# microsoft/protnote

Hardware: AMD Instinct MI355X
Metric: protein-label pairs/sec (fwd+bwd) (higher is better)
Workload: dtype f32

## Files before the change

### include/protnote_hip.h

```cpp
#ifndef PROTNOTE_HIP_H
#define PROTNOTE_HIP_H

#include <stddef.h>
#include <stdint.h>

#ifdef __cplusplus
extern "C" {
#endif

#define PN_MAX_BLOCKS 16
#define PN_MAX_LAYERS 8
#define PN_LABEL_F32 0
#define PN_LABEL_I64 1
#define PN_LABEL_U8 2

const char* pn_last_error(void);
int pn_version(void);
const char* pn_build_hash(void);

typedef struct pn_bn {
  const float* weight;
  const float* bias;
  float* running_mean;
  float* running_var;
// ... 214 lines not shown

int pn_set_mlp_materialize(int on);

typedef int (*pn_sync_hook)(long n_doubles, void* user);
int pn_set_sync_bn(pn_sync_hook hook, void* user, double* stage, long stage_doubles, int world);
int pn_get_math_mode(void);

int pn_set_backward_math(int mode);
int pn_get_backward_math(void);

int pn_set_forward_math(int mode);
int pn_get_forward_math(void);
int pn_set_fwd_staged(int on);
int pn_set_bf16_mfma16(int on);
int pn_set_bwd_deep(int mask);

int pn_set_f32_dma(int on);
int pn_set_b3_dma(int on);

int pn_set_encoder_f64(int on);

int pn_set_conv1_gather(int on);

int pn_dropout_mask(unsigned seed, int stream, float p, long rows, int cols, float* out, void* stream_);

int pn_prof_begin(void);
int pn_prof_end(int max_kinds, int* kinds, long* counts, double* total_ms, double* total_flops);

size_t pn_gemm_nt_stats_ws_bytes(int M, int N);
int pn_gemm_nt(const float* A, long lda, const float* W, long ldw, float* C, long ldc, int M, int N, int K,
// ... 8 lines not shown
```

### protnote_amd/__init__.py

```python
__version__ = "0.1.0"


def free_workspaces():
    from . import _lib

    _lib._ws_cache.clear()


def set_math_mode(mode) -> None:
    from . import _lib

    _lib.set_math_mode(mode)


def get_math_mode() -> str:
    from . import _lib

    return _lib.get_math_mode()


def set_backward_math(mode) -> None:
    from . import _lib

    _lib.set_backward_math(mode)
# ... 5 lines not shown
    return _lib.get_backward_math()


def set_forward_math(mode) -> None:
    from . import _lib

    _lib.set_forward_math(mode)


def get_forward_math() -> str:
    from . import _lib

    return _lib.get_forward_math()


_PROTNOTE_ALIASES = {
    "protnote": "protnote_amd",
    "protnote.models": "protnote_amd.models",
    "protnote.models.ProtNote": "protnote_amd.models.ProtNote",
    "protnote.models.protein_encoders": "protnote_amd.models.protein_encoders",
    "protnote.models.ProtNoteTrainer": "protnote_amd.models.ProtNoteTrainer",
    "protnote.utils": "protnote_amd.utils",
    "protnote.utils.losses": "protnote_amd.utils.losses",
    "protnote.utils.models": "protnote_amd.utils.models",
    "protnote.utils.configs": "protnote_amd.utils.configs",
    "protnote.utils.proteinfer": "protnote_amd.utils.proteinfer",
    "protnote.utils.evaluation": "protnote_amd.utils.evaluation",
    "protnote.data": "protnote_amd.data",
    "protnote.data.collators": "protnote_amd.data.collators",
    "protnote.data.samplers": "protnote_amd.data.samplers",
# ... 22 lines not shown
```

### protnote_amd/_lib.py

```python
import ctypes as C
import os

import torch

_HERE = os.path.dirname(os.path.abspath(__file__))
LIB_PATH = os.path.join(_HERE, "libprotnote_hip.so")

PN_MAX_BLOCKS = 16
PN_MAX_LAYERS = 8
PN_ADAM_WS_BYTES = 32768
fp = C.POINTER(C.c_float)


class pn_bn(C.Structure):
    _fields_ = [("weight", C.c_void_p), ("bias", C.c_void_p), ("running_mean", C.c_void_p),
                ("running_var", C.c_void_p)]


class pn_res_block(C.Structure):
    _fields_ = [("bn1", pn_bn), ("conv_a_w", C.c_void_p), ("conv_a_b", C.c_void_p), ("bn2", pn_bn),
                ("conv_b_w", C.c_void_p), ("conv_b_b", C.c_void_p)]


class pn_encoder(C.Structure):
# ... 142 lines not shown
                                        C.c_void_p, C.c_int, C.c_void_p, C.c_void_p, C.c_void_p]),
    "pn_binned_auprc": (C.c_int, [C.c_void_p, C.c_void_p, C.c_int, C.c_int, C.c_void_p, C.c_void_p, C.c_int,
                                  C.c_void_p]),
    "pn_dropout_mask": (C.c_int, [C.c_uint, C.c_int, C.c_float, C.c_long, C.c_int, C.c_void_p, C.c_void_p]),
    "pn_set_math_mode": (C.c_int, [C.c_int]),
    "pn_set_mlp_materialize": (C.c_int, [C.c_int]),
    "pn_set_sync_bn": (C.c_int, [C.c_void_p, C.c_void_p, C.c_void_p, C.c_long, C.c_int]),
    "pn_get_math_mode": (C.c_int, []),
    "pn_set_backward_math": (C.c_int, [C.c_int]),
    "pn_get_backward_math": (C.c_int, []),
    "pn_set_forward_math": (C.c_int, [C.c_int]),
    "pn_get_forward_math": (C.c_int, []),
    "pn_set_fwd_staged": (C.c_int, [C.c_int]),
    "pn_set_bf16_mfma16": (C.c_int, [C.c_int]),
    "pn_set_bwd_deep": (C.c_int, [C.c_int]),
    "pn_set_f32_dma": (C.c_int, [C.c_int]),
    "pn_set_encoder_f64": (C.c_int, [C.c_int]),
    "pn_set_conv1_gather": (C.c_int, [C.c_int]),
    "pn_set_b3_dma": (C.c_int, [C.c_int]),
    "pn_prof_begin": (C.c_int, []),
    "pn_prof_end": (C.c_int, [C.c_int, C.POINTER(C.c_int), C.POINTER(C.c_long), C.POINTER(C.c_double),
                              C.POINTER(C.c_double)]),
    "pn_gemm_nt": (C.c_int, [C.c_void_p, C.c_long, C.c_void_p, C.c_long, C.c_void_p, C.c_long, C.c_int, C.c_int,
                             C.c_int, C.c_void_p, C.c_void_p, C.c_void_p, C.c_void_p, C.c_void_p, C.c_int,
                             C.c_void_p, C.c_size_t, C.c_void_p]),
    "pn_gemm_nt_stats_ws_bytes": (C.c_size_t, [C.c_int, C.c_int]),
    "pn_loss_ws_bytes": (C.c_size_t, [C.c_int, C.c_int]),
}


# ... 58 lines not shown


def get_math_mode() -> str:
    return "bf16x3" if lib().pn_get_math_mode() == 1 else "f32"


def math_field(mode=None) -> int:
    if mode is None:
        return 1 + int(lib().pn_get_math_mode())
    key = str(mode).lower()
    if key not in _MATH_MODES:
        raise ValueError(f"math mode must be 'f32' or 'bf16x3', got {mode!r}")
    return 1 + _MATH_MODES[key]


_BWD_MODES = {"same": 0, "0": 0, "bf16": 1, "1": 1}


def set_backward_math(mode) -> None:
    key = str(mode).lower()
    if key not in _BWD_MODES:
        raise ValueError(f"backward math must be 'same' or 'bf16', got {mode!r}")
    check(lib().pn_set_backward_math(_BWD_MODES[key]))


def get_backward_math() -> str:
    return "bf16" if lib().pn_get_backward_math() == 1 else "same"


def backward_math_field(mode=None) -> int:
# ... 89 lines not shown
```

### protnote_amd/csrc/abi_heads_train.hpp

```cpp
struct MlpSave {
  float* Y[PN_MAX_LAYERS];
  float* H[PN_MAX_LAYERS];
  float *s[PN_MAX_LAYERS], *t[PN_MAX_LAYERS], *mean[PN_MAX_LAYERS], *invstd[PN_MAX_LAYERS];
};

static bool mlp_save_carve(const pn_mlp* m, int rows, Bump& bp, MlpSave& s) {
  for (int l = 0; l + 1 < m->nlayers; ++l) {
    const int h = m->dims[l + 1];
    s.Y[l] = bp.take<float>((size_t)rows * h);
    s.H[l] = m->dropout_p > 0.f ? bp.take<float>((size_t)rows * h) : nullptr;
    s.s[l] = bp.take<float>(h);
    s.t[l] = bp.take<float>(h);
    s.mean[l] = bp.take<float>(h);
    s.invstd[l] = bp.take<float>(h);
  }
  return bp.ok;
}

struct MlpTrainWs {
  double *S1, *S2;
  float *cs, *p, *q, *G[2], *WT, *part;
  size_t part_floats;
  ColScr colscr;
  StatScr statscr;
// ... 244 lines not shown
struct PairTrainWs {
  double *sumA, *sqA, *sumB, *sqB, *S1, *S2, *dwacc, *scal, *s12;
  float *cs, *p, *q, *WT, *weff, *dweff, *part, *dA1, *dB1;
  float* m1part;
  int m1_chunks;
  float* dwpart;
  long dwpart_rows;
  size_t part_floats;
  ColScr colscr;
  StatScr statscr;
  uint16_t* wsplit;
  int* tnsync;
  uint16_t* hbf;
};
static const long PAIR_STATS_ROWS = 4096;
static const int SUM_BLOCKS = 1024;

static bool pair_train_ws_carve(const pn_pairhead* hd, int B, int NL, Bump& bp, PairTrainWs& w) {
  const int h = hd->h, d = hd->d;
  w.sumA = bp.take<double>(h);
  w.sqA = bp.take<double>(h);
  w.sumB = bp.take<double>(h);
  w.sqB = bp.take<double>(h);
  w.S1 = bp.take<double>(h);
  w.S2 = bp.take<double>(h);
  w.dwacc = bp.take<double>(h);
  w.scal = bp.take<double>(4 + SUM_BLOCKS);
  w.s12 = bp.take<double>(2 * (size_t)h);
  w.cs = bp.take<float>(h);
  w.p = bp.take<float>(h);
  w.q = bp.take<float>(h);
  const size_t wt = (size_t)h * (h > 2 * d ? h : 2 * d);
  w.WT = bp.take<float>(wt);
  w.weff = hd->fusion == 1 ? bp.take<float>((size_t)h * 2 * d) : nullptr;
  w.dweff = hd->fusion == 1 ? bp.take<float>((size_t)h * 2 * d) : nullptr;
  w.part_floats = (size_t)16 * h * h < TN_PART_FLOATS_MAX ? (size_t)16 * h * h : TN_PART_FLOATS_MAX;
  w.part = bp.take<float>(w.part_floats);
  w.dA1 = bp.take<float>((size_t)B * h);
  w.dB1 = bp.take<float>((size_t)NL * h);
  w.m1_chunks = (NL + 255) / 256;
  if (w.m1_chunks < 1) w.m1_chunks = 1;
  if (w.m1_chunks > 128) w.m1_chunks = 128;
  w.m1part = (B <= 256 && hd->fusion != 2) ? bp.take<float>((size_t)w.m1_chunks * B * h) : nullptr;
  w.dwpart_rows = w.m1part != nullptr ? w.m1_chunks : NL;
  w.dwpart = (hd->nlayers == 1 && hd->fusion != 2) ? bp.take<float>((size_t)w.dwpart_rows * h) : nullptr;
  colscr_carve(bp, (long)B * NL, h, w.colscr);
  statscr_carve(bp, (long)B * NL, PAIR_STATS_ROWS, h, w.statscr);
  w.wsplit = (uint16_t*)bp.take<float>((size_t)h * h);
  w.tnsync = bp.take<int>(TN_SYNC_INTS);
  w.hbf = nullptr;
  if (fwd_bf16_requested(hd) && fwd_staged_shape(h) && hd->nlayers > 1) {
    const long R = (long)B * NL;
    w.hbf = (uint16_t*)bp.take<float>((size_t)(R < FWD_H_ROWS ? R : FWD_H_ROWS) * h / 2);
  }
  return bp.ok;
}

static long pair_chunk_rows(int B, int NL, int label_chunk) {
  long c = label_chunk <= 0 ? 256 : label_chunk;
  if (c > NL) c = NL;
  return c * (long)B;
// ... 197 lines not shown
  if (!pair_train_ws_carve(hd, B, NL, bw, w)) return fail("pairhead bwd: workspace too small");

  if (gr->db_out != nullptr) {
    hipLaunchKernelGGL(k_sum, dim3(SUM_BLOCKS), dim3(256), 0, st, dl_pairs, R, w.scal + 4);
    hipLaunchKernelGGL(k_scalar_final, dim3(1), dim3(256), 0, st, (const double*)(w.scal + 4), SUM_BLOCKS, w.scal);
    hipLaunchKernelGGL(k_d2f, dim3(1), dim3(64), 0, st, (const double*)w.scal, gr->db_out, 1, 1.f);
    HIP_OK(hipGetLastError());
  }

  const float* G = nullptr;
  const long stats_rows = PAIR_STATS_ROWS;
  if (hd->backward_math < 0 || hd->backward_math > 2)
    return fail("pairhead bwd: backward_math %d (0 = library default, 1 = as the forward, 2 = bf16)", hd->backward_math);
  const int bwd_math = hd->backward_math == 0 ? g_bwd_math.load(std::memory_order_relaxed) : hd->backward_math - 1;
  BwdBf16Scope bwd_scope(bwd_math == 1 && hd->dropout_p == 0.f);
  for (int l = n - 1; l >= 1; --l) {
    const bool top = (l == n - 1);
    float* z = sv.zbuf[l] + (size_t)S * h;
    StatsParams sp;
    memset(&sp, 0, sizeof(sp));
    sp.R = R; sp.C = h; sp.rows_per_block = stats_rows; sp.pairB = 1;
    sp.Z = z; sp.ldz = h;
    sp.s = sv.s[l]; sp.t = sv.t[l]; sp.mean = sv.mean[l]; sp.invstd = sv.invstd[l];
    sp.part = w.statscr.part;
    const dim3 sg(nblk(h, 1024), nblk(R, stats_rows));
    if (top) {
      sp.gvec = dl_pairs; sp.w = hd->w_out;
      {
        ProfScope ps(ST_BN_BWD_STATS, (double)R * (4.0 * h + 4.0), st);
        hipLaunchKernelGGL((k_bn_bwd_stats<1, 0>), sg, dim3(256), 0, st, sp);
      }
      PN_OK(reduce_parts<double>(w.statscr.part, sg.y, 3 * h, h, w.S1, w.S2, w.dwacc, w.statscr.red, st));
    } else {
      sp.G = G; sp.ldg = h;
      {
        ProfScope ps(ST_BN_BWD_STATS, (double)R * 8.0 * h, st);
        hipLaunchKernelGGL((k_bn_bwd_stats<0, 0>), sg, dim3(256), 0, st, sp);
      }
      PN_OK(reduce_parts<double>(w.statscr.part, sg.y, 2 * h, h, w.S1, w.S2, nullptr, w.statscr.red, st));
    }
    PN_OK(bwd_finalize(st, (const double*)w.S1,
                       (const double*)w.S2, (const double*)(top ? w.dwacc : nullptr), (double)R, h,
                       hd->bn[l].weight, (const float*)sv.s[l], (const float*)sv.mean[l],
                       (const float*)sv.invstd[l], top ? hd->w_out : (const float*)nullptr, w.cs, w.p, w.q,
                       gr->dgamma[l], gr->dbeta[l], top ? gr->dw_out : (float*)nullptr));
    HIP_OK(hipGetLastError());

    const bool dz_bf16 = tl_bwd_bf16 && (g_bwd_deep & 4) && h % 256 == 0 && h <= 4096 && R % 32 == 0 && R >= 65536 &&
// ... 26 lines not shown
    tp.A = dz; tp.lda = h;
    const DropSpec ds_in = drop_spec(hd->dropout_p, hd->dropout_seed, DROP_STREAM_PAIR + (l - 1));
    tp.drop_seed = ds_in.seed; tp.drop_thresh = ds_in.thresh; tp.drop_scale = ds_in.scale;
    if (gr->dw[l] == nullptr) {
    } else if (l == 1 && hd->fusion != 2) {
      tp.B = sv.Ap; tp.ldb = h; tp.B2 = sv.Bp; tp.ldb2 = h; tp.pairB = B;
      PN_OK((launch_tn<TA_PLAIN, TB_PAIRSUM_RELU>(tp, gr->dw[l], h, w.part, w.part_floats, st)));
    } else {
      tp.B = sv.zbuf[l - 1] + (size_t)S * h; tp.ldb = h; tp.b_s = sv.s[l - 1]; tp.b_t = sv.t[l - 1];
      tp.task_sync = w.tnsync;
      PN_OK((launch_tn<TA_PLAIN, TB_AFFINE_RELU>(tp, gr->dw[l], h, w.part, w.part_floats, st)));
    }

    PN_OK(transpose_into(hd->w[l], h, h, h, w.WT, h, st));
    const long step = top ? S : R;
    for (long r0 = 0; r0 < R; r0 += step) {
      const long rows = (R - r0 < step) ? R - r0 : step;
      GemmParams p = gp_zero();
      p.M = (int)rows; p.N = h; p.Nstore = h; p.Kseg = h;
      p.A = dz + (size_t)r0 * h; p.lda = h;
      p.W = w.WT; p.ldw = h; p.wsplit = w.wsplit;
      p.C = sv.zbuf[l] + (size_t)r0 * h; p.ldc = h;
      PN_OK((launch_gemm<A_PLAIN, E_STORE>(p, 0, st)));
    }
    tl_dz_bf16 = false;
    G = sv.zbuf[l];
    if (hd->dropout_p > 0.f)
      PN_OK(launch_dropout<0>(G, h, sv.zbuf[l], h, R, h, nullptr, nullptr, ds_in, st));
  }

  tl_bwd_bf16 = false;
  const bool prod = hd->fusion == 2;
  float* dQ = nullptr;
  if (!prod) {
    PairRedParams rp;
    memset(&rp, 0, sizeof(rp));
    rp.B = B; rp.NL = NL; rp.C = h; rp.DH = G; rp.ldh = h;
    rp.A = sv.A1; rp.lda = h; rp.Bm = sv.B1; rp.ldb = h;
    rp.s = sv.s[0]; rp.t = sv.t[0];
// ... 157 lines not shown
```

### protnote_amd/csrc/gemm_bf16_m16.hpp

```cpp
#pragma once
#include "bwd_bf16_dz.hpp"

namespace pn {

__device__ __forceinline__ void st16(float* ptr, float a, float b, float c, float d) {
  *reinterpret_cast<float4*>(ptr) = make_float4(a, b, c, d);
}

__device__ __forceinline__ float dpp_quad(float v, bool xor2) {
  const int x = __builtin_bit_cast(int, v);
  return __builtin_bit_cast(float, xor2 ? __builtin_amdgcn_update_dpp(x, x, 0x4E, 0xF, 0xF, false)
                                        : __builtin_amdgcn_update_dpp(x, x, 0xB1, 0xF, 0xF, false));
}
__device__ __forceinline__ void quad_transpose(float (&x)[4], int a) {
  const bool o1 = a & 1, o2 = a & 2;
  float r0 = dpp_quad(o1 ? x[0] : x[1], false), r1 = dpp_quad(o1 ? x[2] : x[3], false);
  if (o1) { x[0] = r0; x[2] = r1; } else { x[1] = r0; x[3] = r1; }
  r0 = dpp_quad(o2 ? x[0] : x[2], true);
  r1 = dpp_quad(o2 ? x[1] : x[3], true);
  if (o2) { x[0] = r0; x[1] = r1; } else { x[2] = r0; x[3] = r1; }
}

template <int EK, int WAVES_M, int WAVES_N, int FM, int FN>
__device__ __forceinline__ void gemm_epilogue_m16(const GemmParams& p, f32x4 (&acc)[FM][FN], int row0, int col0, int tile_n, float* smem) {
  static_assert(EK == E_STORE || EK == E_ROWDOT, "E_STORE_H16 takes the swapped roles");
  static_assert(FN % 4 == 0, "stores transpose four fragments at a time");
  constexpr int NT = WAVES_M * WAVES_N * 64;
  constexpr int BN = WAVES_N * FN * 16;
  const int tid = threadIdx.x;
  const int lane = tid & 63;
  const int wave = tid >> 6;
  const int wm = wave / WAVES_N;
  const int wn = wave % WAVES_N;
  const int rq = lane >> 4;
  const int cl = lane & 15;
  const int qa = lane & 3, qc = cl >> 2;
  const bool want_stats = (EK == E_STORE) && (p.col_part != nullptr);
  const bool store_act = (EK == E_STORE) && (p.e_scale != nullptr);
  float* red = smem;

  if constexpr (EK == E_ROWDOT) {
    float rowacc[FM][4];
#pragma unroll
    for (int i = 0; i < FM; ++i)
#pragma unroll
      for (int e = 0; e < 4; ++e) rowacc[i][e] = 0.f;
#pragma unroll
    for (int j = 0; j < FN; ++j) {
      const int col = col0 + (wn * FN + j) * 16 + cl;
      const float es = p.e_scale[col], et = p.e_shift[col], ew = p.e_w[col];
#pragma unroll
      for (int i = 0; i < FM; ++i)
// ... 7 lines not shown
        float v = rowacc[i][e];
        v += __shfl_xor(v, 1);
        v += __shfl_xor(v, 2);
        v += __shfl_xor(v, 4);
        v += __shfl_xor(v, 8);
        const int row = row0 + (wm * FM + i) * 16 + 4 * rq + e;
        if (cl == 0 && row < p.M) p.rowdot_out[(long)(tile_n * WAVES_N + wn) * p.M + row] = v;
      }
    }
    return;
  } else {
#pragma unroll
    for (int j = 0; j < FN; ++j) {
      const int col = col0 + (wn * FN + j) * 16 + cl;
      float bj = 0.f, es = 1.f, et = 0.f;
      if constexpr (EK == E_STORE) bj = p.bias ? p.bias[col] : 0.f;
      const bool act = store_act;
      if (act) {
        es = p.e_scale[col];
        et = p.e_shift[col];
      }
      float s1 = 0.f, s2 = 0.f;
#pragma unroll
      for (int i = 0; i < FM; ++i) {
#pragma unroll
        for (int e = 0; e < 4; ++e) {
          float v = acc[i][j][e];
          if constexpr (EK == E_STORE) v += bj;
          if (act) v = relu(fmaf(v, es, et));
          acc[i][j][e] = v;
          const int row = row0 + (wm * FM + i) * 16 + 4 * rq + e;
          if (row < p.M) {
            s1 += v;
            s2 += v * v;
          }
        }
      }
      if (want_stats) {
        s1 += __shfl_xor(s1, 16);
        s2 += __shfl_xor(s2, 16);
        s1 += __shfl_xor(s1, 32);
        s2 += __shfl_xor(s2, 32);
        if (rq == 0) {
          red[(wm * 2 + 0) * BN + (wn * FN + j) * 16 + cl] = s1;
          red[(wm * 2 + 1) * BN + (wn * FN + j) * 16 + cl] = s2;
        }
      }
    }
#pragma unroll
    for (int i = 0; i < FM; ++i) {
#pragma unroll
      for (int e = 0; e < 4; ++e) {
// ... 190 lines not shown
```

### protnote_amd/csrc/gemm_engine.hpp

```cpp
#pragma once
#include <hip/hip_runtime.h>
#include <stdint.h>

#include <type_traits>

#ifndef PN_MINW
#define PN_MINW 2
#endif
#ifndef PN_BK
#define PN_BK 32
#endif
#ifndef PN_XCD
#define PN_XCD 1
#endif

namespace pn {

typedef float f32x16 __attribute__((ext_vector_type(16)));

enum { A_PLAIN = 0, A_AFFINE_RELU = 1, A_PAIRSUM_RELU = 2, A_CONV = 3, A_DZ_ELEM = 4, A_DZ_ROWG = 5, A_PAIRPROD = 6 };
enum { E_STORE = 0, E_CONV = 1, E_ROWDOT = 2, E_SCALE_RC = 3, E_PAIRADD = 4, E_STORE_H16 = 5 };

struct GemmParams {
  int M, N;
  int Nstore;
  int nseg, Kseg;
  const float* A;
  long lda;
  const float* a_scale;
  const float* a_shift;
  const float* A2;
  long lda2;
  int pairB;
  const int* lens;
  int L;
  int dil;
// ... 17 lines not shown
  float alpha;
  const float* gvec;
  const float* dz_cs;
  const float* dz_p;
  const float* dz_q;
  const float* padd1;
  long ldp1;
  const float* padd2;
  long ldp2;
  uint32_t drop_seed, drop_thresh;
  float drop_scale;
  uint16_t* wsplit;
  const uint16_t* w_hi;
  const uint16_t* w_lo;
  int xcd_br, xcd_bc;
  const int* run_if;
};

__device__ __forceinline__ float4 ld4(const float* p) { return *reinterpret_cast<const float4*>(p); }
__device__ __forceinline__ float relu(float x) { return fmaxf(x, 0.f); }

__host__ __device__ __forceinline__ uint32_t pn_lowbias32(uint32_t x) {
  x ^= x >> 16;
  x *= 0x7feb352dU;
  x ^= x >> 15;
  x *= 0x846ca68bU;
  x ^= x >> 16;
  return x;
}
__host__ __device__ __forceinline__ uint32_t drop_rowkey(uint32_t seed, uint32_t row) {
// ... 37 lines not shown
  return true;
}

template <int EK, int WAVES_M, int WAVES_N, int WM, int WN>
__device__ __forceinline__ void gemm_epilogue(const GemmParams& p, f32x16 (&acc)[WM][WN], int row0, int col0, int tile_n,
                                              float* smem) {
  constexpr int NT = WAVES_M * WAVES_N * 64;
  constexpr int BN = WAVES_N * WN * 32;
  const int tid = threadIdx.x;
  const int lane = tid & 63;
  const int wave = tid >> 6;
  const int wm = wave / WAVES_N;
  const int wn = wave % WAVES_N;
  const int hl = lane >> 5;
  const int cl = lane & 31;
  const bool want_stats = (EK == E_STORE || EK == E_CONV || EK == E_PAIRADD) && (p.col_part != nullptr);
  float* red = smem;

  unsigned live_mask[WM];
  if constexpr (EK == E_CONV) {
#pragma unroll
    for (int i = 0; i < WM; ++i) {
      live_mask[i] = 0u;
#pragma unroll
      for (int e = 0; e < 16; ++e) {
        const int row = row0 + (wm * WM + i) * 32 + (e & 3) + 8 * (e >> 2) + 4 * hl;
        const int rc = row < p.M ? row : p.M - 1;
        const int b = rc / p.L;
        const bool live = (row < p.M) && (rc - b * p.L) < p.lens[b];
        live_mask[i] |= (live ? 1u : 0u) << e;
      }
    }
  }

#pragma unroll
  for (int j = 0; j < WN; ++j) {
    const int col = col0 + (wn * WN + j) * 32 + cl;
    const bool cok = col < p.N;
    float s1 = 0.f, s2 = 0.f;
    float bj = 0.f, es = 0.f, et = 0.f, ew = 0.f, cs = 0.f;
    if constexpr (EK == E_STORE || EK == E_CONV || EK == E_PAIRADD) {
      bj = (cok && p.bias) ? p.bias[col] : 0.f;
    }
    if constexpr (EK == E_ROWDOT) {
      if (cok) {
        es = p.e_scale[col];
        et = p.e_shift[col];
        ew = p.e_w[col];
      }
    }
    if constexpr (EK == E_STORE_H16) {
      if (cok) {
        es = p.e_scale[col];
        et = p.e_shift[col];
      }
    }
    const bool store_act = (EK == E_STORE) && (p.e_scale != nullptr);
// ... 16 lines not shown
          const int rc = row < p.M ? row : p.M - 1;
          res[e] = has_res ? p.resid[(long)rc * p.ldr + cc] : 0.f;
        }
#pragma unroll
        for (int e = 0; e < 16; ++e) {
          const int row = row0 + (wm * WM + i) * 32 + (e & 3) + 8 * (e >> 2) + 4 * hl;
          const bool live = (live_mask[i] >> e) & 1u;
          float v = acc[i][j][e];
          v = (live && cok) ? (v + bj) + res[e] : 0.f;
          if (row < p.M && col < p.Nstore) p.C[(long)row * p.ldc + col] = v;
          s1 += v;
          s2 += v * v;
        }
      }
    }
    if constexpr (EK != E_CONV) {
#pragma unroll
    for (int i = 0; i < WM; ++i) {
#pragma unroll
      for (int e = 0; e < 16; ++e) {
        const int row = row0 + (wm * WM + i) * 32 + (e & 3) + 8 * (e >> 2) + 4 * hl;
        const bool rok = row < p.M;
        float v = acc[i][j][e];
        if constexpr (EK == E_PAIRADD) {
          if (rok && cok) {
            const int pj = row / p.pairB;
            const int pi = row - pj * p.pairB;
            v += bj + p.padd1[(long)pi * p.ldp1 + col] + p.padd2[(long)pj * p.ldp2 + col];
            p.C[(long)row * p.ldc + col] = v;
            s1 += v;
            s2 += v * v;
// ... 350 lines not shown
```

### protnote_amd/csrc/protnote_hip.hip

```cpp
#include <hip/hip_runtime.h>
#include <stdarg.h>
#include <stdio.h>
#include <stdlib.h>
#include <string.h>

#include "../../include/protnote_hip.h"
#include "common.hpp"
#include "gemm_engine.hpp"
#include "gemm_bf16x3.hpp"
#include "gemm_bf16.hpp"
#include "gemm_dma.hpp"
#include "gemm_conv_dma.hpp"
#include "gemm_conv_f64.hpp"
#include "gemm_tn_fast.hpp"
#include "train_kernels.hpp"
#include "bwd_bf16_dz.hpp"
#include "fwd_bf16_h.hpp"
#include "gemm_bf16_m16.hpp"

using namespace pn;

static thread_local char g_err[512] = "";

static int fail(const char* fmt, ...) {
// ... 233 lines not shown
  *count_dev = nullptr;
  if (!sync_bn_on()) return 0;
  if (2 * n + 2 > g_sync_cap) return fail("sync_bn: %ld statistics exceed the staging buffer (%ld doubles)", 2 * n + 2, g_sync_cap);
  HIP_OK(hipMemcpyAsync(g_sync_stage, a, n * sizeof(double), hipMemcpyDeviceToDevice, st));
  HIP_OK(hipMemcpyAsync(g_sync_stage + n, b, n * sizeof(double), hipMemcpyDeviceToDevice, st));
  hipLaunchKernelGGL(k_set_double, dim3(1), dim3(1), 0, st, g_sync_stage + 2 * n, local_count);
  if (g_sync_hook(2 * n + 1, g_sync_user) != 0) return fail("sync_bn: the all-reduce callback failed");
  HIP_OK(hipMemcpyAsync(a, g_sync_stage, n * sizeof(double), hipMemcpyDeviceToDevice, st));
  HIP_OK(hipMemcpyAsync(b, g_sync_stage + n, n * sizeof(double), hipMemcpyDeviceToDevice, st));
  double* keep = g_sync_stage + g_sync_cap - 1;
  HIP_OK(hipMemcpyAsync(keep, g_sync_stage + 2 * n, sizeof(double), hipMemcpyDeviceToDevice, st));
  *count_dev = keep;
  return 0;
}

template <int AK, int EK, int WAVES_M, int WAVES_N, int WM, int WN, int BK, bool DROP = false>
static int launch_gemm_cfg(const GemmParams& p, hipStream_t st) {
  using Cfg = GemmCfg<WAVES_M, WAVES_N, WM, WN, BK>;
  auto kern = gemm_nt_kernel<AK, EK, WAVES_M, WAVES_N, WM, WN, BK, DROP>;
  static std::atomic<bool> attr_done[64];
  int dev = 0;
  HIP_OK(hipGetDevice(&dev));
  if (dev < 64 && !attr_done[dev]) {
    HIP_OK(hipFuncSetAttribute((const void*)kern, hipFuncAttributeMaxDynamicSharedMemorySize,
                               Cfg::LDS_BYTES));
    attr_done[dev] = true;
  }
  if (p.M <= 0 || p.Nstore <= 0) return 0;
  if (p.Kseg % 4 != 0) return fail("gemm: K segment %d not a multiple of 4", p.Kseg);
  const long tm = (p.M + Cfg::BM - 1) / Cfg::BM;
  const long tn = (p.Nstore + Cfg::BN - 1) / Cfg::BN;
  if (tm * tn > 0x7fffffffL) return fail("gemm: grid too large");
  GemmParams pp = p;
  const int resident = (Cfg::BM * Cfg::BN >= 256 * 256) ? 32 : 64;
  pp.xcd_bc = (PN_XCD && tm >= 16) ? ((tn % 8 == 0) ? 8 : ((tn % 4 == 0) ? 4 : 0)) : 0;
  if (AK == A_PAIRSUM_RELU && resident == 32 && pp.xcd_bc && tm >= 64) pp.xcd_bc = 1;
  pp.xcd_br = pp.xcd_bc ? resident / pp.xcd_bc : 0;
  long grid = tm * tn;
  if (pp.xcd_bc) {
    const long nblk = ((tm + pp.xcd_br - 1) / pp.xcd_br) * (tn / pp.xcd_bc);
    grid = ((nblk + 7) / 8) * 8 * resident;
  }
  if (grid > 0x7fffffffL) return fail("gemm: grid too large");
  {
    ProfScope ps(AK * 10 + EK, 2.0 * (double)p.M * (double)p.N * (double)p.nseg * (double)p.Kseg, st);
    hipLaunchKernelGGL(kern, dim3((unsigned)grid), dim3(Cfg::NT), Cfg::LDS_BYTES, st, pp);
  }
  HIP_OK(hipGetLastError());
  return finish_col_stats(p, tm, st);
}

static std::atomic<int> g_math_mode{0};
extern "C" int pn_set_math_mode(int mode) {
  if (mode != 0 && mode != 1) return fail("pn_set_math_mode: 0 (f32) or 1 (bf16x3)");
  g_math_mode = mode;
  return 0;
}
extern "C" int pn_get_math_mode(void) { return g_math_mode; }
static thread_local int tl_math = -1;
static inline int cur_math() { return tl_math >= 0 ? tl_math : g_math_mode.load(std::memory_order_relaxed); }
// ... 77 lines not shown
  }
  if (p.M <= 0 || p.Nstore <= 0) return 0;
  if (p.Kseg % 4 != 0) return fail("gemm: K segment %d not a multiple of 4", p.Kseg);
  const long tm = (p.M + Cfg::BM - 1) / Cfg::BM;
  const long tn = (p.Nstore + Cfg::BN - 1) / Cfg::BN;
  GemmParams pp = p;
  pp.xcd_bc = (PN_XCD && tm >= 16) ? ((tn % 8 == 0) ? 8 : ((tn % 4 == 0) ? 4 : 0)) : 0;
  if (!GEN && AK == A_PAIRSUM_RELU && pp.xcd_bc && tm >= 64) pp.xcd_bc = 1;
  pp.xcd_br = pp.xcd_bc ? 32 / pp.xcd_bc : 0;
  long grid = tm * tn;
  if (pp.xcd_bc) {
    const long nblk = ((tm + pp.xcd_br - 1) / pp.xcd_br) * (tn / pp.xcd_bc);
    grid = ((nblk + 7) / 8) * 8 * 32;
  }
  if (grid > 0x7fffffffL) return fail("gemm: grid too large");
  if constexpr (BDMA) {
    pp.w_hi = p.wsplit;
    pp.w_lo = p.wsplit + (size_t)p.N * p.Kseg;
    hipLaunchKernelGGL(k_split_planes, dim3(nblk((long)p.N * p.Kseg / 4, 256)), dim3(256), 0, st, p.W, p.ldw, p.N, p.Kseg,
                       p.wsplit, p.wsplit + (size_t)p.N * p.Kseg);
  }
  {
    ProfScope ps((NP == 3 ? 1000 : 1500) + AK * 10 + EK, 2.0 * (double)p.M * (double)p.N * (double)p.nseg * (double)p.Kseg, st);
    hipLaunchKernelGGL(kern, dim3((unsigned)grid), dim3(Cfg::NT), LDS_BYTES, st, pp);
  }
  HIP_OK(hipGetLastError());
  return finish_col_stats(p, tm, st);
}

static std::atomic<int> g_bwd_deep{7};
extern "C" int pn_set_bwd_deep(int mask) {
  g_bwd_deep = mask & 7;
  return 0;
}
static int launch_gemm_bf16_single(const GemmParams& p, hipStream_t st) {
  auto kern = gemm_nt_bf16_kernel<E_STORE>;
  static std::atomic<bool> attr_done[64];
  int dev = 0;
  HIP_OK(hipGetDevice(&dev));
  if (dev < 64 && !attr_done[dev]) {
    HIP_OK(hipFuncSetAttribute((const void*)kern, hipFuncAttributeMaxDynamicSharedMemorySize, NT_BF16_LDS_BYTES));
    attr_done[dev] = true;
  }
  if (p.M <= 0 || p.Nstore <= 0) return 0;
  const long tm = (p.M + 255) / 256, tn = p.N / 256;
  GemmParams pp = p;
  pp.xcd_bc = (PN_XCD && tm >= 16) ? ((tn % 8 == 0) ? 8 : ((tn % 4 == 0) ? 4 : 0)) : 0;
  pp.xcd_br = pp.xcd_bc ? 32 / pp.xcd_bc : 0;
  long grid = tm * tn;
  if (pp.xcd_bc) {
    const long nblk_ = ((tm + pp.xcd_br - 1) / pp.xcd_br) * (tn / pp.xcd_bc);
    grid = ((nblk_ + 7) / 8) * 8 * 32;
  }
  if (grid > 0x7fffffffL) return fail("gemm: grid too large");
  pp.w_hi = p.wsplit;
  pp.w_lo = p.wsplit + (size_t)p.N * p.Kseg;
  hipLaunchKernelGGL(k_split_planes, dim3(nblk((long)p.N * p.Kseg / 4, 256)), dim3(256), 0, st, p.W, p.ldw, p.N, p.Kseg,
                     p.wsplit, p.wsplit + (size_t)p.N * p.Kseg);
  {
    ProfScope ps(1500 + A_PLAIN * 10 + E_STORE, 2.0 * (double)p.M * (double)p.N * (double)p.Kseg, st);
    hipLaunchKernelGGL(kern, dim3((unsigned)grid), dim3(512), NT_BF16_LDS_BYTES, st, pp);
  }
  HIP_OK(hipGetLastError());
  return 0;
}

static std::atomic<int> g_bf16_m16{1};
extern "C" int pn_set_bf16_mfma16(int on) {
  g_bf16_m16 = on ? 1 : 0;
  return 0;
}
template <int EK>
static int bf16dma_kernel(void (**out)(GemmParams)) {
  static std::atomic<bool> attr_done[64];
  int dev = 0;
  HIP_OK(hipGetDevice(&dev));
  if (dev < 64 && !attr_done[dev]) {
    HIP_OK(hipFuncSetAttribute((const void*)gemm_nt_bf16dma_kernel<EK>, hipFuncAttributeMaxDynamicSharedMemorySize, NT_BF16DMA_LDS_BYTES));
    HIP_OK(hipFuncSetAttribute((const void*)gemm_nt_bf16m16_kernel<EK>, hipFuncAttributeMaxDynamicSharedMemorySize, NT_BF16DMA_LDS_BYTES));
    attr_done[dev] = true;
  }
  *out = g_bf16_m16.load() ? gemm_nt_bf16m16_kernel<EK> : gemm_nt_bf16dma_kernel<EK>;
  return 0;
}

static int launch_gemm_bf16dma(const GemmParams& p, hipStream_t st) {
  void (*kern)(GemmParams) = nullptr;
  if (int rc = bf16dma_kernel<E_STORE>(&kern)) return rc;
  if (p.M <= 0 || p.Nstore <= 0) return 0;
  if (p.wsplit == nullptr || p.Kseg % 64 != 0 || p.N % 256 != 0 || p.Nstore != p.N || (long)256 * p.lda * 4 >= (1L << 32) ||
      (long)256 * p.Kseg * 2 >= (1L << 32))
    return fail("gemm (bf16 dz): shape %d x %d x %d not supported", p.M, p.N, p.Kseg);
  const long tm = (p.M + 255) / 256, tn = p.N / 256;
  GemmParams pp = p;
  pp.xcd_bc = (PN_XCD && tm >= 16) ? ((tn % 8 == 0) ? 8 : ((tn % 4 == 0) ? 4 : 0)) : 0;
  pp.xcd_br = pp.xcd_bc ? 32 / pp.xcd_bc : 0;
  long grid = tm * tn;
  if (pp.xcd_bc) {
    const long nblk_ = ((tm + pp.xcd_br - 1) / pp.xcd_br) * (tn / pp.xcd_bc);
    grid = ((nblk_ + 7) / 8) * 8 * 32;
  }
  if (grid > 0x7fffffffL) return fail("gemm: grid too large");
  pp.w_hi = p.wsplit;
  hipLaunchKernelGGL(k_round_plane, dim3(nblk((long)p.N * p.Kseg / 4, 256)), dim3(256), 0, st, p.W, p.ldw, p.N, p.Kseg, p.wsplit);
  {
    ProfScope ps(1500 + A_PLAIN * 10 + E_STORE, 2.0 * (double)p.M * (double)p.N * (double)p.Kseg, st);
    hipLaunchKernelGGL(kern, dim3((unsigned)grid), dim3(512), NT_BF16DMA_LDS_BYTES, st, pp);
  }
  HIP_OK(hipGetLastError());
  return 0;
}

#ifndef PN_BIG
#define PN_BIG 1
#endif
static std::atomic<int> g_fwd_staged{1};
extern "C" int pn_set_fwd_staged(int on) {
// ... 80 lines not shown
    HIP_OK(hipFuncSetAttribute((const void*)kern, hipFuncAttributeMaxDynamicSharedMemorySize, GEMM_DMA_LDS_BYTES));
    attr_done[dev] = true;
  }
  if (p.M <= 0 || p.Nstore <= 0) return 0;
  const long tm = (p.M + 255) / 256, tn = p.N / 256;
  GemmParams pp = p;
  pp.xcd_bc = (PN_XCD && tm >= 16) ? ((tn % 8 == 0) ? 8 : ((tn % 4 == 0) ? 4 : 0)) : 0;
  if (AK == A_PAIRSUM_RELU && pp.xcd_bc && tm >= 64) pp.xcd_bc = 1;
  pp.xcd_br = pp.xcd_bc ? 32 / pp.xcd_bc : 0;
  long grid = tm * tn;
  if (pp.xcd_bc) {
    const long nblk_ = ((tm + pp.xcd_br - 1) / pp.xcd_br) * (tn / pp.xcd_bc);
    grid = ((nblk_ + 7) / 8) * 8 * 32;
  }
  if (grid > 0x7fffffffL) return fail("gemm: grid too large");
  {
    ProfScope ps(AK * 10 + EK, 2.0 * (double)p.M * (double)p.N * (double)p.Kseg, st);
    hipLaunchKernelGGL(kern, dim3((unsigned)grid), dim3(512), GEMM_DMA_LDS_BYTES, st, pp);
  }
  HIP_OK(hipGetLastError());
  return finish_col_stats(p, tm, st);
}

static int launch_conv_dma(const GemmParams& p, int Lp, int ktrue, hipStream_t st) {
  constexpr int WN = 3;
  auto kern = gemm_conv_dma_kernel<WN>;
  constexpr int LDS = conv_dma_lds_bytes<WN>();
  static std::atomic<bool> attr_done[64];
  int dev = 0;
  HIP_OK(hipGetDevice(&dev));
  if (dev < 64 && !attr_done[dev]) {
    HIP_OK(hipFuncSetAttribute((const void*)kern, hipFuncAttributeMaxDynamicSharedMemorySize, LDS));
// ... 24 lines not shown
static int rowdot_nparts(int n);
#ifndef PN_BIG
#define PN_BIG 1
#endif
template <int AK>
static bool dma_offsets_fit(const GemmParams& p) {
  const long lim = 1L << 32;
  if ((long)256 * p.lda * 4 >= lim || (long)256 * p.ldw * 4 >= lim) return false;
  if (AK == A_PAIRSUM_RELU)
    return p.pairB > 0 && p.lda2 % 4 == 0 && (long)p.pairB * p.lda * 4 < lim && ((long)p.M / p.pairB + 1) * p.lda2 * 4 < lim;
  return true;
}

template <int AK, int EK>
static int launch_gemm(const GemmParams& p, int variant, hipStream_t st) {
  if (p.drop_thresh != 0) {
    if constexpr ((AK == A_AFFINE_RELU || AK == A_PAIRSUM_RELU) && EK == E_STORE) {
      if (PN_BIG && use_f32_dma() && variant == 0 && p.M >= 65536 && p.nseg == 1 && p.Kseg % 32 == 0 && p.N % 256 == 0 &&
          p.Nstore == p.N && p.lda % 4 == 0 && p.ldw % 4 == 0 && dma_offsets_fit<AK>(p))
        return launch_gemm_dma<AK, EK, true>(p, st);
      return launch_gemm_cfg<AK, EK, 2, 2, 2, 2, PN_BK, true>(p, st);
    } else {
      return fail("gemm: dropout is not defined for operand kind %d / epilogue %d", AK, EK);
    }
  }
  if (tl_fwd_bf16 && PN_BIG) {
    if constexpr ((AK == A_PLAIN || AK == A_AFFINE_RELU || AK == A_PAIRSUM_RELU) && (EK == E_STORE || EK == E_ROWDOT)) {
      if (variant == 0 && p.nseg == 1 && p.Kseg % 32 == 0 && p.N % 256 == 0 && p.Nstore == p.N && p.wsplit != nullptr &&
          p.lda % 4 == 0 && (AK != A_PAIRSUM_RELU || p.lda2 % 4 == 0))
        return launch_gemm_bf16x3<AK, EK, 2, 4, false, true, 1>(p, st);
    }
  }
  if (tl_bwd_bf16 && PN_BIG) {
    if constexpr (AK == A_PLAIN && EK == E_STORE) {
      if (tl_dz_bf16) return launch_gemm_bf16dma(p, st);
      if (variant == 0 && p.M >= 4096 && p.nseg == 1 && p.Kseg % 32 == 0 && p.N % 256 == 0 && p.Nstore == p.N &&
          p.wsplit != nullptr && p.bias == nullptr && p.e_scale == nullptr && p.col_part == nullptr) {
        if ((g_bwd_deep & 1) && p.Kseg >= 96 && (long)256 * p.lda * 4 < (1L << 32) && p.lda % 4 == 0)
          return launch_gemm_bf16_single(p, st);
        return launch_gemm_bf16x3<AK, EK, 2, 4, false, true, 1>(p, st);
      }
    }
  }
  if (cur_math() == 1 && PN_BIG) {
    if constexpr ((AK == A_PLAIN || AK == A_AFFINE_RELU || AK == A_PAIRSUM_RELU) && (EK == E_STORE || EK == E_ROWDOT)) {
      if (variant == 0 && p.M >= 65536 && p.nseg == 1 && p.Kseg % 32 == 0 && p.N % 256 == 0 && p.Nstore == p.N)
        return launch_gemm_bf16x3<AK, EK, 2, 4, false>(p, st);
    }
    if constexpr ((AK == A_PLAIN || AK == A_AFFINE_RELU) && EK == E_STORE) {
      if (variant == 0 && p.M >= 8192 && p.N >= 512) return launch_gemm_bf16x3<AK, EK, 2, 4, true>(p, st);
    }
    if constexpr (AK == A_CONV && EK == E_CONV) {
      if (variant == 3) return launch_gemm_bf16x3<AK, EK, 2, 3, true>(p, st);
    }
  }
  if constexpr ((AK == A_PLAIN || AK == A_AFFINE_RELU || AK == A_PAIRSUM_RELU) && (EK == E_STORE || EK == E_ROWDOT)) {
    if (PN_BIG && use_f32_dma() && (variant == 0 || EK == E_ROWDOT) && p.M >= g_dma_min_rows && p.nseg == 1 && p.Kseg % 32 == 0 &&
        p.N % 256 == 0 && p.Nstore == p.N && p.lda % 4 == 0 && p.ldw % 4 == 0 && dma_offsets_fit<AK>(p))
      return launch_gemm_dma<AK, EK>(p, st);
  }
  if constexpr ((EK == E_STORE && (AK == A_PLAIN || AK == A_AFFINE_RELU || AK == A_PAIRSUM_RELU)) ||
                (EK == E_PAIRADD && AK == A_PAIRPROD)) {
    if (PN_BIG && variant == 0 && p.N % 256 == 0 && p.M >= 65536)
      return launch_gemm_cfg<AK, EK, 4, 2, 2, 4, 32>(p, st);
  }
  if constexpr (EK == E_CONV) {
    if (PN_BIG && variant == 3) return launch_gemm_cfg<AK, EK, 4, 2, 2, 3, 32>(p, st);
  }
  if constexpr (EK == E_ROWDOT) {
    if (PN_BIG && p.N % 256 == 0) return launch_gemm_cfg<AK, EK, 4, 2, 2, 4, 32>(p, st);
  }
  if (variant == 1) return launch_gemm_cfg<AK, EK, 4, 1, 1, 2, PN_BK>(p, st);
  return launch_gemm_cfg<AK, EK, 2, 2, 2, 2, PN_BK>(p, st);
}

static int rowdot_nparts(int n) {
// ... 242 lines not shown
```

Measured before the change: 1.256 million.

## Fuse BatchNorm-backward column statistics into pair-head backward GEMM epilogue

```diff
diff --git a/include/protnote_hip.h b/include/protnote_hip.h
--- a/include/protnote_hip.h
+++ b/include/protnote_hip.h
@@ -252,6 +252,7 @@
 int pn_set_fwd_staged(int on);
 int pn_set_bf16_mfma16(int on);
 int pn_set_bwd_deep(int mask);
+int pn_set_bn_bwd_fused(int on);
 
 int pn_set_f32_dma(int on);
 int pn_set_b3_dma(int on);
diff --git a/protnote_amd/__init__.py b/protnote_amd/__init__.py
--- a/protnote_amd/__init__.py
+++ b/protnote_amd/__init__.py
@@ -43,6 +43,12 @@
     return _lib.get_forward_math()
 
 
+def set_bn_bwd_fused(on) -> None:
+    from . import _lib
+
+    _lib.set_bn_bwd_fused(on)
+
+
 _PROTNOTE_ALIASES = {
     "protnote": "protnote_amd",
     "protnote.models": "protnote_amd.models",
diff --git a/protnote_amd/_lib.py b/protnote_amd/_lib.py
--- a/protnote_amd/_lib.py
+++ b/protnote_amd/_lib.py
@@ -180,6 +180,7 @@
     "pn_set_fwd_staged": (C.c_int, [C.c_int]),
     "pn_set_bf16_mfma16": (C.c_int, [C.c_int]),
     "pn_set_bwd_deep": (C.c_int, [C.c_int]),
+    "pn_set_bn_bwd_fused": (C.c_int, [C.c_int]),
     "pn_set_f32_dma": (C.c_int, [C.c_int]),
     "pn_set_encoder_f64": (C.c_int, [C.c_int]),
     "pn_set_conv1_gather": (C.c_int, [C.c_int]),
@@ -268,6 +269,10 @@
     return 1 + _MATH_MODES[key]
 
 
+def set_bn_bwd_fused(on) -> None:
+    check(lib().pn_set_bn_bwd_fused(1 if on else 0))
+
+
 _BWD_MODES = {"same": 0, "0": 0, "bf16": 1, "1": 1}
 
 
diff --git a/protnote_amd/csrc/abi_heads_train.hpp b/protnote_amd/csrc/abi_heads_train.hpp
--- a/protnote_amd/csrc/abi_heads_train.hpp
+++ b/protnote_amd/csrc/abi_heads_train.hpp
@@ -282,6 +282,7 @@
   uint16_t* hbf;
 };
 static const long PAIR_STATS_ROWS = 4096;
+static const long PAIR_DBN_SLACK_ROWS = 64 * 128;
 static const int SUM_BLOCKS = 1024;
 
 static bool pair_train_ws_carve(const pn_pairhead* hd, int B, int NL, Bump& bp, PairTrainWs& w) {
@@ -312,7 +313,7 @@
   w.m1part = (B <= 256 && hd->fusion != 2) ? bp.take<float>((size_t)w.m1_chunks * B * h) : nullptr;
   w.dwpart_rows = w.m1part != nullptr ? w.m1_chunks : NL;
   w.dwpart = (hd->nlayers == 1 && hd->fusion != 2) ? bp.take<float>((size_t)w.dwpart_rows * h) : nullptr;
-  colscr_carve(bp, (long)B * NL, h, w.colscr);
+  colscr_carve(bp, (long)B * NL + PAIR_DBN_SLACK_ROWS, h, w.colscr);
   statscr_carve(bp, (long)B * NL, PAIR_STATS_ROWS, h, w.statscr);
   w.wsplit = (uint16_t*)bp.take<float>((size_t)h * h);
   w.tnsync = bp.take<int>(TN_SYNC_INTS);
@@ -540,6 +541,7 @@
     return fail("pairhead bwd: backward_math %d (0 = library default, 1 = as the forward, 2 = bf16)", hd->backward_math);
   const int bwd_math = hd->backward_math == 0 ? g_bwd_math.load(std::memory_order_relaxed) : hd->backward_math - 1;
   BwdBf16Scope bwd_scope(bwd_math == 1 && hd->dropout_p == 0.f);
+  bool stats_done = false;
   for (int l = n - 1; l >= 1; --l) {
     const bool top = (l == n - 1);
     float* z = sv.zbuf[l] + (size_t)S * h;
@@ -557,7 +559,7 @@
         hipLaunchKernelGGL((k_bn_bwd_stats<1, 0>), sg, dim3(256), 0, st, sp);
       }
       PN_OK(reduce_parts<double>(w.statscr.part, sg.y, 3 * h, h, w.S1, w.S2, w.dwacc, w.statscr.red, st));
-    } else {
+    } else if (!stats_done) {
       sp.G = G; sp.ldg = h;
       {
         ProfScope ps(ST_BN_BWD_STATS, (double)R * 8.0 * h, st);
@@ -614,6 +616,14 @@
 
     PN_OK(transpose_into(hd->w[l], h, h, h, w.WT, h, st));
     const long step = top ? S : R;
+    const long dbn_slots = ((long)B * NL + PAIR_DBN_SLACK_ROWS + 127) / 128;
+    bool dbn = g_bn_bwd_fused.load(std::memory_order_relaxed) == 1 && l >= 2 && hd->dropout_p == 0.f;
+    if (dbn) {
+      long need = 0;
+      for (long r0 = 0; r0 < R; r0 += step) need += (((R - r0 < step) ? R - r0 : step) + 127) / 128;
+      dbn = need <= dbn_slots;
+    }
+    long tiles = 0;
     for (long r0 = 0; r0 < R; r0 += step) {
       const long rows = (R - r0 < step) ? R - r0 : step;
       GemmParams p = gp_zero();
@@ -621,8 +631,19 @@
       p.A = dz + (size_t)r0 * h; p.lda = h;
       p.W = w.WT; p.ldw = h; p.wsplit = w.wsplit;
       p.C = sv.zbuf[l] + (size_t)r0 * h; p.ldc = h;
-      PN_OK((launch_gemm<A_PLAIN, E_STORE>(p, 0, st)));
-    }
+      if (dbn) {
+        p.col_part = w.colscr.part + (size_t)tiles * 2 * h;
+        p.dbn_slots = (int)(dbn_slots - tiles);
+        p.dbn_z = sv.zbuf[l - 1] + (size_t)(S + r0) * h; p.dbn_ldz = h;
+        p.dbn_s = sv.s[l - 1]; p.dbn_t = sv.t[l - 1]; p.dbn_mean = sv.mean[l - 1]; p.dbn_invstd = sv.invstd[l - 1];
+        PN_OK((launch_gemm<A_PLAIN, E_STORE_DBN>(p, 0, st)));
+        tiles += tl_gemm_row_tiles;
+      } else {
+        PN_OK((launch_gemm<A_PLAIN, E_STORE>(p, 0, st)));
+      }
+    }
+    if (dbn) PN_OK(reduce_parts<float>(w.colscr.part, tiles, 2 * h, h, w.S1, w.S2, nullptr, w.colscr.red, st));
+    stats_done = dbn;
     tl_dz_bf16 = false;
     G = sv.zbuf[l];
     if (hd->dropout_p > 0.f)
diff --git a/protnote_amd/csrc/gemm_bf16_m16.hpp b/protnote_amd/csrc/gemm_bf16_m16.hpp
--- a/protnote_amd/csrc/gemm_bf16_m16.hpp
+++ b/protnote_amd/csrc/gemm_bf16_m16.hpp
@@ -23,7 +23,7 @@
 
 template <int EK, int WAVES_M, int WAVES_N, int FM, int FN>
 __device__ __forceinline__ void gemm_epilogue_m16(const GemmParams& p, f32x4 (&acc)[FM][FN], int row0, int col0, int tile_n, float* smem) {
-  static_assert(EK == E_STORE || EK == E_ROWDOT, "E_STORE_H16 takes the swapped roles");
+  static_assert(EK == E_STORE || EK == E_ROWDOT || EK == E_STORE_DBN, "E_STORE_H16 takes the swapped roles");
   static_assert(FN % 4 == 0, "stores transpose four fragments at a time");
   constexpr int NT = WAVES_M * WAVES_N * 64;
   constexpr int BN = WAVES_N * FN * 16;
@@ -35,7 +35,7 @@
   const int rq = lane >> 4;
   const int cl = lane & 15;
   const int qa = lane & 3, qc = cl >> 2;
-  const bool want_stats = (EK == E_STORE) && (p.col_part != nullptr);
+  const bool want_stats = (EK == E_STORE || EK == E_STORE_DBN) && (p.col_part != nullptr);
   const bool store_act = (EK == E_STORE) && (p.e_scale != nullptr);
   float* red = smem;
 
@@ -73,13 +73,35 @@
     for (int j = 0; j < FN; ++j) {
       const int col = col0 + (wn * FN + j) * 16 + cl;
       float bj = 0.f, es = 1.f, et = 0.f;
-      if constexpr (EK == E_STORE) bj = p.bias ? p.bias[col] : 0.f;
+      if constexpr (EK == E_STORE || EK == E_STORE_DBN) bj = p.bias ? p.bias[col] : 0.f;
       const bool act = store_act;
       if (act) {
         es = p.e_scale[col];
         et = p.e_shift[col];
       }
       float s1 = 0.f, s2 = 0.f;
+      if constexpr (EK == E_STORE_DBN) {
+        const float ds = p.dbn_s[col], dt = p.dbn_t[col], dmu = p.dbn_mean[col], dis = p.dbn_invstd[col];
+        float zr[FM][4];
+#pragma unroll
+        for (int i = 0; i < FM; ++i)
+#pragma unroll
+          for (int e = 0; e < 4; ++e) {
+            const int row = row0 + (wm * FM + i) * 16 + 4 * rq + e;
+            zr[i][e] = p.dbn_z[(long)(row < p.M ? row : p.M - 1) * p.dbn_ldz + col];
+          }
+#pragma unroll
+        for (int i = 0; i < FM; ++i)
+#pragma unroll
+          for (int e = 0; e < 4; ++e) {
+            const float v = acc[i][j][e] + bj;
+            acc[i][j][e] = v;
+            const int row = row0 + (wm * FM + i) * 16 + 4 * rq + e;
+            const float u = (row < p.M && fmaf(zr[i][e], ds, dt) > 0.f) ? v : 0.f;
+            s1 += u;
+            s2 = fmaf(u, (zr[i][e] - dmu) * dis, s2);
+          }
+      } else {
 #pragma unroll
       for (int i = 0; i < FM; ++i) {
 #pragma unroll
@@ -95,6 +117,7 @@
           }
         }
       }
+      }
       if (want_stats) {
         s1 += __shfl_xor(s1, 16);
         s2 += __shfl_xor(s2, 16);
diff --git a/protnote_amd/csrc/gemm_engine.hpp b/protnote_amd/csrc/gemm_engine.hpp
--- a/protnote_amd/csrc/gemm_engine.hpp
+++ b/protnote_amd/csrc/gemm_engine.hpp
@@ -19,7 +19,7 @@
 typedef float f32x16 __attribute__((ext_vector_type(16)));
 
 enum { A_PLAIN = 0, A_AFFINE_RELU = 1, A_PAIRSUM_RELU = 2, A_CONV = 3, A_DZ_ELEM = 4, A_DZ_ROWG = 5, A_PAIRPROD = 6 };
-enum { E_STORE = 0, E_CONV = 1, E_ROWDOT = 2, E_SCALE_RC = 3, E_PAIRADD = 4, E_STORE_H16 = 5 };
+enum { E_STORE = 0, E_CONV = 1, E_ROWDOT = 2, E_SCALE_RC = 3, E_PAIRADD = 4, E_STORE_H16 = 5, E_STORE_DBN = 6 };
 
 struct GemmParams {
   int M, N;
@@ -67,6 +67,13 @@
   const uint16_t* w_hi;
   const uint16_t* w_lo;
   int xcd_br, xcd_bc;
+  const float* dbn_z;
+  long dbn_ldz;
+  const float* dbn_s;
+  const float* dbn_t;
+  const float* dbn_mean;
+  const float* dbn_invstd;
+  int dbn_slots;
   const int* run_if;
 };
 
@@ -134,7 +141,7 @@
   const int wn = wave % WAVES_N;
   const int hl = lane >> 5;
   const int cl = lane & 31;
-  const bool want_stats = (EK == E_STORE || EK == E_CONV || EK == E_PAIRADD) && (p.col_part != nullptr);
+  const bool want_stats = (EK == E_STORE || EK == E_CONV || EK == E_PAIRADD || EK == E_STORE_DBN) && (p.col_part != nullptr);
   float* red = smem;
 
   unsigned live_mask[WM];
@@ -159,8 +166,32 @@
     const bool cok = col < p.N;
     float s1 = 0.f, s2 = 0.f;
     float bj = 0.f, es = 0.f, et = 0.f, ew = 0.f, cs = 0.f;
-    if constexpr (EK == E_STORE || EK == E_CONV || EK == E_PAIRADD) {
+    if constexpr (EK == E_STORE || EK == E_CONV || EK == E_PAIRADD || EK == E_STORE_DBN) {
       bj = (cok && p.bias) ? p.bias[col] : 0.f;
+    }
+    if constexpr (EK == E_STORE_DBN) {
+      const int cc = cok ? col : 0;
+      const float ds = p.dbn_s[cc], dt = p.dbn_t[cc], dmu = p.dbn_mean[cc], dis = p.dbn_invstd[cc];
+#pragma unroll
+      for (int i = 0; i < WM; ++i) {
+        float zr[16];
+#pragma unroll
+        for (int e = 0; e < 16; ++e) {
+          const int row = row0 + (wm * WM + i) * 32 + (e & 3) + 8 * (e >> 2) + 4 * hl;
+          const int rc = row < p.M ? row : p.M - 1;
+          zr[e] = p.dbn_z[(long)rc * p.dbn_ldz + cc];
+        }
+#pragma unroll
+        for (int e = 0; e < 16; ++e) {
+          const int row = row0 + (wm * WM + i) * 32 + (e & 3) + 8 * (e >> 2) + 4 * hl;
+          const bool rok = row < p.M;
+          const float v = cok ? acc[i][j][e] + bj : 0.f;
+          if (rok && col < p.Nstore) p.C[(long)row * p.ldc + col] = v;
+          const float u = (rok && cok && fmaf(zr[e], ds, dt) > 0.f) ? v : 0.f;
+          s1 += u;
+          s2 = fmaf(u, (zr[e] - dmu) * dis, s2);
+        }
+      }
     }
     if constexpr (EK == E_ROWDOT) {
       if (cok) {
@@ -207,7 +238,7 @@
         }
       }
     }
-    if constexpr (EK != E_CONV) {
+    if constexpr (EK != E_CONV && EK != E_STORE_DBN) {
 #pragma unroll
     for (int i = 0; i < WM; ++i) {
 #pragma unroll
diff --git a/protnote_amd/csrc/protnote_hip.hip b/protnote_amd/csrc/protnote_hip.hip
--- a/protnote_amd/csrc/protnote_hip.hip
+++ b/protnote_amd/csrc/protnote_hip.hip
@@ -271,6 +271,21 @@
   return 0;
 }
 
+static thread_local long tl_gemm_row_tiles = 0;
+template <int EK>
+static int dbn_check(const GemmParams& p, long tm) {
+  tl_gemm_row_tiles = tm;
+  if constexpr (EK == E_STORE_DBN) {
+    if (p.col_part == nullptr || p.dbn_z == nullptr || p.dbn_s == nullptr || p.dbn_t == nullptr || p.dbn_mean == nullptr ||
+        p.dbn_invstd == nullptr)
+      return fail("gemm: the BatchNorm-backward epilogue needs col_part, dbn_z and the four column vectors");
+    if (tm > (long)p.dbn_slots) return fail("gemm: %ld row tiles of BatchNorm-backward partials, %d slots", tm, p.dbn_slots);
+  }
+  return 0;
+}
+template <int EK>
+constexpr int prof_ek() { return EK == E_STORE_DBN ? (int)E_STORE : EK; }
+
 template <int AK, int EK, int WAVES_M, int WAVES_N, int WM, int WN, int BK, bool DROP = false>
 static int launch_gemm_cfg(const GemmParams& p, hipStream_t st) {
   using Cfg = GemmCfg<WAVES_M, WAVES_N, WM, WN, BK>;
@@ -299,8 +314,9 @@
     grid = ((nblk + 7) / 8) * 8 * resident;
   }
   if (grid > 0x7fffffffL) return fail("gemm: grid too large");
+  PN_OK(dbn_check<EK>(p, tm));
   {
-    ProfScope ps(AK * 10 + EK, 2.0 * (double)p.M * (double)p.N * (double)p.nseg * (double)p.Kseg, st);
+    ProfScope ps(AK * 10 + prof_ek<EK>(), 2.0 * (double)p.M * (double)p.N * (double)p.nseg * (double)p.Kseg, st);
     hipLaunchKernelGGL(kern, dim3((unsigned)grid), dim3(Cfg::NT), Cfg::LDS_BYTES, st, pp);
   }
   HIP_OK(hipGetLastError());
@@ -408,6 +424,7 @@
     grid = ((nblk + 7) / 8) * 8 * 32;
   }
   if (grid > 0x7fffffffL) return fail("gemm: grid too large");
+  PN_OK(dbn_check<EK>(p, tm));
   if constexpr (BDMA) {
     pp.w_hi = p.wsplit;
     pp.w_lo = p.wsplit + (size_t)p.N * p.Kseg;
@@ -415,7 +432,7 @@
                        p.wsplit, p.wsplit + (size_t)p.N * p.Kseg);
   }
   {
-    ProfScope ps((NP == 3 ? 1000 : 1500) + AK * 10 + EK, 2.0 * (double)p.M * (double)p.N * (double)p.nseg * (double)p.Kseg, st);
+    ProfScope ps((NP == 3 ? 1000 : 1500) + AK * 10 + prof_ek<EK>(), 2.0 * (double)p.M * (double)p.N * (double)p.nseg * (double)p.Kseg, st);
     hipLaunchKernelGGL(kern, dim3((unsigned)grid), dim3(Cfg::NT), LDS_BYTES, st, pp);
   }
   HIP_OK(hipGetLastError());
@@ -427,8 +444,9 @@
   g_bwd_deep = mask & 7;
   return 0;
 }
+template <int EK>
 static int launch_gemm_bf16_single(const GemmParams& p, hipStream_t st) {
-  auto kern = gemm_nt_bf16_kernel<E_STORE>;
+  auto kern = gemm_nt_bf16_kernel<EK>;
   static std::atomic<bool> attr_done[64];
   int dev = 0;
   HIP_OK(hipGetDevice(&dev));
@@ -447,6 +465,7 @@
     grid = ((nblk_ + 7) / 8) * 8 * 32;
   }
   if (grid > 0x7fffffffL) return fail("gemm: grid too large");
+  PN_OK(dbn_check<EK>(p, tm));
   pp.w_hi = p.wsplit;
   pp.w_lo = p.wsplit + (size_t)p.N * p.Kseg;
   hipLaunchKernelGGL(k_split_planes, dim3(nblk((long)p.N * p.Kseg / 4, 256)), dim3(256), 0, st, p.W, p.ldw, p.N, p.Kseg,
@@ -462,6 +481,11 @@
 static std::atomic<int> g_bf16_m16{1};
 extern "C" int pn_set_bf16_mfma16(int on) {
   g_bf16_m16 = on ? 1 : 0;
+  return 0;
+}
+static std::atomic<int> g_bn_bwd_fused{1};
+extern "C" int pn_set_bn_bwd_fused(int on) {
+  g_bn_bwd_fused = on ? 1 : 0;
   return 0;
 }
 template <int EK>
@@ -478,9 +502,10 @@
   return 0;
 }
 
+template <int EK>
 static int launch_gemm_bf16dma(const GemmParams& p, hipStream_t st) {
   void (*kern)(GemmParams) = nullptr;
-  if (int rc = bf16dma_kernel<E_STORE>(&kern)) return rc;
+  if (int rc = bf16dma_kernel<EK>(&kern)) return rc;
   if (p.M <= 0 || p.Nstore <= 0) return 0;
   if (p.wsplit == nullptr || p.Kseg % 64 != 0 || p.N % 256 != 0 || p.Nstore != p.N || (long)256 * p.lda * 4 >= (1L << 32) ||
       (long)256 * p.Kseg * 2 >= (1L << 32))
@@ -495,6 +520,7 @@
     grid = ((nblk_ + 7) / 8) * 8 * 32;
   }
   if (grid > 0x7fffffffL) return fail("gemm: grid too large");
+  PN_OK(dbn_check<EK>(p, tm));
   pp.w_hi = p.wsplit;
   hipLaunchKernelGGL(k_round_plane, dim3(nblk((long)p.N * p.Kseg / 4, 256)), dim3(256), 0, st, p.W, p.ldw, p.N, p.Kseg, p.wsplit);
   {
@@ -605,8 +631,9 @@
     grid = ((nblk_ + 7) / 8) * 8 * 32;
   }
   if (grid > 0x7fffffffL) return fail("gemm: grid too large");
+  PN_OK(dbn_check<EK>(p, tm));
   {
-    ProfScope ps(AK * 10 + EK, 2.0 * (double)p.M * (double)p.N * (double)p.Kseg, st);
+    ProfScope ps(AK * 10 + prof_ek<EK>(), 2.0 * (double)p.M * (double)p.N * (double)p.Kseg, st);
     hipLaunchKernelGGL(kern, dim3((unsigned)grid), dim3(512), GEMM_DMA_LDS_BYTES, st, pp);
   }
   HIP_OK(hipGetLastError());
@@ -661,6 +688,8 @@
 
 template <int AK, int EK>
 static int launch_gemm(const GemmParams& p, int variant, hipStream_t st) {
+  static_assert(EK != E_STORE_DBN || AK == A_PLAIN, "E_STORE_DBN: plain operand only");
+  constexpr bool STORE = (EK == E_STORE || EK == E_STORE_DBN);
   if (p.drop_thresh != 0) {
     if constexpr ((AK == A_AFFINE_RELU || AK == A_PAIRSUM_RELU) && EK == E_STORE) {
       if (PN_BIG && use_f32_dma() && variant == 0 && p.M >= 65536 && p.nseg == 1 && p.Kseg % 32 == 0 && p.N % 256 == 0 &&
@@ -672,41 +701,41 @@
     }
   }
   if (tl_fwd_bf16 && PN_BIG) {
-    if constexpr ((AK == A_PLAIN || AK == A_AFFINE_RELU || AK == A_PAIRSUM_RELU) && (EK == E_STORE || EK == E_ROWDOT)) {
+    if constexpr ((AK == A_PLAIN || AK == A_AFFINE_RELU || AK == A_PAIRSUM_RELU) && (STORE || EK == E_ROWDOT)) {
       if (variant == 0 && p.nseg == 1 && p.Kseg % 32 == 0 && p.N % 256 == 0 && p.Nstore == p.N && p.wsplit != nullptr &&
           p.lda % 4 == 0 && (AK != A_PAIRSUM_RELU || p.lda2 % 4 == 0))
         return launch_gemm_bf16x3<AK, EK, 2, 4, false, true, 1>(p, st);
     }
   }
   if (tl_bwd_bf16 && PN_BIG) {
-    if constexpr (AK == A_PLAIN && EK == E_STORE) {
-      if (tl_dz_bf16) return launch_gemm_bf16dma(p, st);
+    if constexpr (AK == A_PLAIN && STORE) {
+      if (tl_dz_bf16) return launch_gemm_bf16dma<EK>(p, st);
       if (variant == 0 && p.M >= 4096 && p.nseg == 1 && p.Kseg % 32 == 0 && p.N % 256 == 0 && p.Nstore == p.N &&
-          p.wsplit != nullptr && p.bias == nullptr && p.e_scale == nullptr && p.col_part == nullptr) {
+          p.wsplit != nullptr && p.bias == nullptr && p.e_scale == nullptr && (EK == E_STORE_DBN || p.col_part == nullptr)) {
         if ((g_bwd_deep & 1) && p.Kseg >= 96 && (long)256 * p.lda * 4 < (1L << 32) && p.lda % 4 == 0)
-          return launch_gemm_bf16_single(p, st);
+          return launch_gemm_bf16_single<EK>(p, st);
         return launch_gemm_bf16x3<AK, EK, 2, 4, false, true, 1>(p, st);
       }
     }
   }
   if (cur_math() == 1 && PN_BIG) {
-    if constexpr ((AK == A_PLAIN || AK == A_AFFINE_RELU || AK == A_PAIRSUM_RELU) && (EK == E_STORE || EK == E_ROWDOT)) {
+    if constexpr ((AK == A_PLAIN || AK == A_AFFINE_RELU || AK == A_PAIRSUM_RELU) && (STORE || EK == E_ROWDOT)) {
       if (variant == 0 && p.M >= 65536 && p.nseg == 1 && p.Kseg % 32 == 0 && p.N % 256 == 0 && p.Nstore == p.N)
         return launch_gemm_bf16x3<AK, EK, 2, 4, false>(p, st);
     }
-    if constexpr ((AK == A_PLAIN || AK == A_AFFINE_RELU) && EK == E_STORE) {
+    if constexpr ((AK == A_PLAIN || AK == A_AFFINE_RELU) && STORE) {
       if (variant == 0 && p.M >= 8192 && p.N >= 512) return launch_gemm_bf16x3<AK, EK, 2, 4, true>(p, st);
     }
     if constexpr (AK == A_CONV && EK == E_CONV) {
       if (variant == 3) return launch_gemm_bf16x3<AK, EK, 2, 3, true>(p, st);
     }
   }
-  if constexpr ((AK == A_PLAIN || AK == A_AFFINE_RELU || AK == A_PAIRSUM_RELU) && (EK == E_STORE || EK == E_ROWDOT)) {
+  if constexpr ((AK == A_PLAIN || AK == A_AFFINE_RELU || AK == A_PAIRSUM_RELU) && (STORE || EK == E_ROWDOT)) {
     if (PN_BIG && use_f32_dma() && (variant == 0 || EK == E_ROWDOT) && p.M >= g_dma_min_rows && p.nseg == 1 && p.Kseg % 32 == 0 &&
         p.N % 256 == 0 && p.Nstore == p.N && p.lda % 4 == 0 && p.ldw % 4 == 0 && dma_offsets_fit<AK>(p))
       return launch_gemm_dma<AK, EK>(p, st);
   }
-  if constexpr ((EK == E_STORE && (AK == A_PLAIN || AK == A_AFFINE_RELU || AK == A_PAIRSUM_RELU)) ||
+  if constexpr ((STORE && (AK == A_PLAIN || AK == A_AFFINE_RELU || AK == A_PAIRSUM_RELU)) ||
                 (EK == E_PAIRADD && AK == A_PAIRPROD)) {
     if (PN_BIG && variant == 0 && p.N % 256 == 0 && p.M >= 65536)
       return launch_gemm_cfg<AK, EK, 4, 2, 2, 4, 32>(p, st);
```

Result: no change. 1.249 million (-0.5%).
